# saugns/saugns

Hardware: AMD Instinct MI355X
Metric: mono samples/sec/GPU @ N voices (depth-3 FM) (higher is better)
Workload: dtype f32 (f64 table interpolation, u32 phase)

## Files before the change

### __graft_entry__.py

```python
import os
import subprocess
import sys

ROOT = os.path.dirname(os.path.abspath(__file__))
if ROOT not in sys.path:
    sys.path.insert(0, ROOT)


def build():
    import saugns_amd
    saugns_amd.build(force=False)
    subprocess.check_call(["make", "-s", "-C", os.path.join(ROOT, "tests", "seqexec")])
    subprocess.check_call(["make", "-s", "-C", os.path.join(ROOT, "tests", "hooks")])
    subprocess.check_call(["make", "-s", "-C", os.path.join(ROOT, "tests", "hooks_levels")])
    subprocess.check_call(["make", "-s", "-C", os.path.join(ROOT, "oracle"), "oracle"])
    subprocess.check_call(["make", "-s", "-C", os.path.join(ROOT, "oracle"), "ref"])
    subprocess.check_call(["make", "-s", "-C", os.path.join(ROOT, "oracle"), "hosts"])
    saugns_amd.lib()


def smoke():
    import numpy as np
    import saugns_amd as sa
    from saugns_amd import voicebank
    from oracle import pyoracle as po

    tabs = np.fromfile(os.path.join(ROOT, "tests", "golden", "piluts_ref.f32"),
                       dtype="<f4").reshape(12, 2048)
    sa.set_piluts(tabs)
    po.oracle_use_tables(tabs)
    po.oracle().ora_set_fastmath_forms(1)
    prg = voicebank.config3(n=16, seconds=1)
    want = po.oracle_render(prg.ptr, 44100, False)
    got = sa.Generator(prg, 44100).render(stereo=False)
    assert len(got) == len(want) == 44100, (len(got), len(want))
    diff = int(np.abs(got.astype(np.int32) - want.astype(np.int32)).max())
    assert diff == 0, f"GPU render differs from the oracle by {diff} LSB"
    print("smoke ok: 16 voices x depth-3 PM, 44100 frames, bit-exact vs oracle")
    from saugns_amd.api import POP_FMOD
    fm = [voicebank.Op("sin", freq=voicebank.Line(110.0 + 20 * k, goal=330.0, shape="exp"), time_ms=500,
                       mods={POP_FMOD: [voicebank.Op("sin", freq=5.0 + k, amp=20.0)]}) for k in range(8)]
    for name, p in (("8 FM voices with gliding carriers", voicebank.build_program(fm)),
                    ("16 feedback voices (config 5)", voicebank.config5(n=16, seconds=1))):
        want = po.oracle_render(p.ptr, 44100, False)
        got = sa.Generator(p, 44100).render(stereo=False)
        assert len(got) == len(want) and (got == want).all(), name
        print(f"smoke ok: {name}, {len(got)} frames, bit-exact vs oracle")


if __name__ == "__main__":
    build()
    if "--smoke" in sys.argv:
        smoke()
```

### saugns_amd/csrc/hip_backend.hip

```cpp
#include <hip/hip_runtime.h>
#include "hip_backend.h"
#include "launch_plan.h"
#include "sau_dev_ops.h"
#include <stdio.h>
#include <stdlib.h>
#include <string.h>
#include <deque>
#include <map>
#include <mutex>
#include <string>
#include <type_traits>
#include <vector>

namespace sauhip {

using namespace saudev;
using sauengine::BackendConfig;
using sauengine::tune_env;
using sauengine::SegmentDesc;
using namespace sauplan;

#include "k_common.h"
#include "k_block_loop.h"
#include "k_fast_types.h"
// ... 681 lines not shown
		if (getenv("SAU_AMD_DEBUG_DUO"))
			fprintf(stderr, "[sau-amd] duo %d: enabled %d look %d words_real %u FT %u rows_cf %u cub_ok %u tail %d may_scan %u of %u voices, lds %zu of %zu\n",
					(int)k.duo, (int)tun_.duo, fp.look != nullptr, fp.look_words_real, k.rows, k.rows_cf, fp.cub_ok, (int)j.tail_live, seg.n_may_scan, seg.n_voices,
					k.launch_lds(2, k.rows, false) + 1024, lim_.lds_limit);
		cfp.dyn_chunks = k.tasks_cf.dyn_chunks; cfp.dyn_static = k.tasks_cf.dyn_static;
		if (!k.duo && !launch_build(j, err, 0, k.rows_cf, k.grid_cf, &cfp, true, k.wide_cf)) j.launched = false;
		fp.mode = fp.sum_levels + 1; fp.only_multi = 0; fp.look_wpv = k.look_wpv; fp.look_groups = k.groups;
		fp.look_wpv_flags = k.look_wpv_flags;
		if (k.duo) {
			const size_t dlds = k.launch_lds(2, k.rows, false);
			if (!raise_lds_attr((const void *)duo_kernel, dlds, dev_, err)) return false;
			auto go = [&]() -> bool {
				void *da[] = {(void *)&fp, (void *)&cfp};
				return hipLaunchKernel((const void *)duo_kernel, dim3(lim_.fk_grid), dim3(1024), da, dlds, stream_) == hipSuccess;
			};
			if (!SpreadLaunchOrder::get().ordered(dev_, stream_, go)) j.launched = false;
		} else if (fp.look) {
			if (k.look_inside) {
				if (!launch_build(j, err, 2, k.rows, k.grid_look, nullptr, false, k.wide_look)) j.launched = false;
			} else if (!SpreadLaunchOrder::get().ordered(dev_, stream_, [&]() { return launch_build(j, err, 2, k.rows, k.grid_look, nullptr, false, k.wide_look); })) {
				j.launched = false;
			}
			if (fp.cub_ok) {
				const void *ck2 = fast_kernel_fn(2, FAST_CUB_ROWS, FK_CUB);
				const size_t lds2 = k.launch_lds(2, FAST_CUB_ROWS, false);
				if (!raise_lds_attr(ck2, lds2, dev_, err)) return false;
				auto go = [&]() -> bool {
					void *a2[] = {(void *)&fp};
					return hipLaunchKernel(ck2, dim3(k.grid_look), dim3(1024), a2, lds2, stream_) == hipSuccess;
				};
				if (k.look_inside ? !go() : !SpreadLaunchOrder::get().ordered(dev_, stream_, go)) j.launched = false;
			}
		}
		return true;
	}

	bool launch_sums_and_chains(Job &j, std::string &err) {
		const SegmentDesc &seg = j.seg;
		FastParams &fp = j.fp;
		if (fp.chain_rows && fp.chain_early_ok && !launch_early_chains(j, err)) return false;
		for (uint32_t pass = 1; pass <= fp.sum_levels && (!fp.look || seg.n_chain_rows); ++pass) {
			launch_fast(j, err, pass);
			hipLaunchKernelGGL(scan_kernel, dim3(seg.n_voices), dim3(64), 0, stream_, fp);
		}
		if (!fp.chain_rows) { launch_fast(j, err, fp.sum_levels + 1); return true; }
		return launch_chains(j, err);
	}

	bool launch_early_chains(Job &j, std::string &err) {
		FastParams &fp = j.fp;
		const uint32_t cgrid = j.fk.chain_grid;
		const size_t clds = chain_alone_lds((size_t)fp.n_ctabs * CHAIN_TAB_BYTES + CHAIN_IO_BYTES, cgrid);
		if (!raise_lds_attr((const void *)chain_kernel, clds, dev_, err)) return false;
		fp.chain_early = 1; fp.range_mode = 0;
		hipLaunchKernelGGL(chain_kernel, dim3(cgrid), dim3(192), clds, stream_, fp);
		const size_t rlds = chain_alone_lds(RCHAIN_LDS_BYTES, cgrid);
		if (!raise_lds_attr((const void *)rchain_kernel, rlds, dev_, err)) return false;
		hipLaunchKernelGGL(rchain_kernel, dim3(cgrid), dim3(RCHAIN_THREADS), rlds, stream_, fp);
		fp.chain_early = 0;
		return true;
	}

	bool launch_chains(Job &j, std::string &err) {
		const FastPlan &k = j.fk;
		FastParams &fp = j.fp;
		const uint32_t cgrid = k.chain_grid, n_chunks = k.chunks.n;
		const size_t clds = chain_alone_lds((size_t)fp.n_ctabs * CHAIN_TAB_BYTES + CHAIN_IO_BYTES, cgrid);
		if (!raise_lds_attr((const void *)chain_kernel, clds, dev_, err)) return false;
		TimedPair *tc = nullptr;
		if (n_chunks == 1) {
			tc = timing_on_ ? new_pair(0) : nullptr;
			fp.range_mode = 0;
			launch_fast(j, err, fp.sum_levels + 2);
			if (tc) (void)hipEventRecord(tc->a, stream_);
			hipLaunchKernelGGL(chain_kernel, dim3(cgrid), dim3(192), clds, stream_, fp);
			if (tc) (void)hipEventRecord(tc->b, stream_);
			launch_fast(j, err, fp.sum_levels + 1);
			return true;
		}
		if (!chain_stream_) {
			chain_stream_ = StreamPool::get().take(dev_, 1);
			if (!chain_stream_) {
				int lo = 0, hi = 0;
				(void)hipDeviceGetStreamPriorityRange(&lo, &hi);
				HIP_OK(hipStreamCreateWithPriority(&chain_stream_, hipStreamNonBlocking, hi));
			}
		}
		while (chain_ev_.size() < 2 * (size_t)n_chunks) {
			hipEvent_t e;
			HIP_OK(hipEventCreateWithFlags(&e, hipEventDisableTiming));
			chain_ev_.push_back(e);
		}
		tc = timing_on_ ? new_pair(0) : nullptr;
		const uint32_t *cb = k.chunks.cb;
		auto set_range = [&](FastParams &q, uint32_t mode, uint32_t c) {
			q.range_mode = mode; q.f_lo = cb[c]; q.f_hi = c + 1 == n_chunks ? 0xffffffffu : cb[c + 1];
		};
		for (uint32_t c = 0; c < n_chunks; ++c) {
			set_range(fp, 1, c);
			fp.range_last = c + 1 == n_chunks;
			launch_fast(j, err, fp.sum_levels + 2, k.pass_grid);
			HIP_OK(hipEventRecord(chain_ev_[2 * c], stream_));
			HIP_OK(hipStreamWaitEvent(chain_stream_, chain_ev_[2 * c], 0));
			FastParams cp = fp;
			set_range(cp, 1, c);
			if (tc && c == 0) (void)hipEventRecord(tc->a, chain_stream_);
			hipLaunchKernelGGL(chain_kernel, dim3(cgrid), dim3(192), clds, chain_stream_, cp);
			if (tc && c + 1 == n_chunks) (void)hipEventRecord(tc->b, chain_stream_);
			HIP_OK(hipEventRecord(chain_ev_[2 * c + 1], chain_stream_));
		}
		uint32_t mixed_blocks = 0;
		if (k.early_mix) hipLaunchKernelGGL(premix_kernel, dim3((j.seg.n_voices + 63) / 64), dim3(64), 0, stream_, fp);
		for (uint32_t c = 0; c < n_chunks; ++c) {
			HIP_OK(hipStreamWaitEvent(stream_, chain_ev_[2 * c + 1], 0));
			set_range(fp, 2, c);
			fp.range_last = c + 1 == n_chunks;
			launch_fast(j, err, fp.sum_levels + 1, c + 1 == n_chunks ? k.grid : k.pass_grid);
			if (k.early_mix && c + 1 < n_chunks && cb[c + 1] > 512) {
				const uint32_t hi = (cb[c + 1] - 512) / 256;
				if (hi > mixed_blocks) {
					MixParams mp = mix_params(j.seg, set_);
					mp.blk_lo = mixed_blocks; mp.blk_hi = hi;
					TimedPair *tm = timing_on_ ? new_pair(1) : nullptr;
					if (tm) (void)hipEventRecord(tm->a, stream_);
					hipLaunchKernelGGL((j.in.f32 ? mix_kernel_f32 : mix_kernel), dim3(hi - mixed_blocks, j.seg.n_streams), dim3(256), 0, stream_, mp);
					if (tm) (void)hipEventRecord(tm->b, stream_);
					mixed_blocks = hi;
				}
			}
		}
		j.early_mixed_blocks = mixed_blocks;
		fp.range_mode = 0; fp.f_lo = 0; fp.f_hi = 0; fp.range_last = 0;
		return true;
	}

	bool launch_closed_form(Job &j, std::string &err) {
		const SegmentDesc &seg = j.seg;
		const FastPlan &k = j.fk;
		FastParams &fp = j.fp;
		fp.dyn_chunks = k.tasks.dyn_chunks; fp.dyn_static = k.tasks.dyn_static; fp.dyn_small = k.tasks.dyn_small;
		if (k.queues) {
			fp.inmix_flags = k.inmix_flags;
			fp.inmix_div_s = k.div.s; fp.inmix_div_m = k.div.m;
			if (k.inmix) {
				fp.inmix_stream = set_.mstreams.p;
				fp.inmix_pcm_offset = seg.pcm_offset;
				hipLaunchKernelGGL(premix_kernel, dim3((seg.n_voices + 63) / 64), dim3(64), 0, stream_, fp);
				j.inmix_live = true;
			}
		}
		if (k.inner != INNER_NONE) {
			const bool lm = k.inner == INNER_LANE_MAJOR;
			const void *ik = fast_kernel_fn(0, 12, FK_WIDE | FK_INNER | (lm ? FK_LANEMAJOR : 0u));
			const size_t lds = k.launch_lds(0, k.rows, true);
			FastParams ep = fp;
			ep.mode = 0; ep.edge_only = 1; ep.dyn_static = 1; ep.dyn_chunks = 2; ep.dyn_small = 0; ep.inmix_flags = 0;
			if (!launch_build(j, err, 0, k.rows, k.grid_edge, &ep, false, true)) j.launched = false;
			fp.mode = 0;
			void *iargs[] = {(void *)&fp};
			if (!raise_lds_attr(ik, lds, dev_, err)) return false;
			HIP_OK(hipLaunchKernel(ik, dim3(k.grid), dim3(1024), iargs, lds, stream_));
			if (inner_report_) fprintf(stderr, "[sau-amd] inner: %s, %u voices\n", lm ? "lane-major" : "row-major", seg.n_voices);
		} else {
			if (inner_report_) fprintf(stderr, "[sau-amd] inner: none (rows %u, wide %d, chunks %u), %u voices\n", k.rows, k.wide_cf ? 1 : 0, fp.dyn_chunks, seg.n_voices);
			launch_fast(j, err, 0);
		}
		fp.dyn_chunks = 0; fp.inmix_flags = 0; fp.dyn_small = 0;
		return true;
	}

	bool launch_cub(Job &j, std::string &err) {
		if (!j.fp.cub_ok) return true;
		const FastPlan &k = j.fk;
		FastParams q = k.main_build == 2 ? j.cfp : j.fp;
		q.n_fast = k.n_fast_cf; q.rows = FAST_CUB_ROWS; q.mode = 0; q.only_multi = 0;
		q.dyn_chunks = k.tasks_cub.dyn_chunks; q.dyn_static = k.tasks_cub.dyn_static;
		const size_t qlds = k.launch_lds(0, FAST_CUB_ROWS, false, true);
		const void *ck = fast_kernel_fn(0, FAST_CUB_ROWS, FK_CUB);
		if (!raise_lds_attr(ck, qlds, dev_, err)) return false;
		void *qargs[] = {(void *)&q};
		HIP_OK(hipLaunchKernel(ck, dim3(k.grid_cub), dim3(1024), qargs, qlds, stream_));
		return true;
	}

	bool launch_repair(Job &j, std::string &err) {
		const FastPlan &k = j.fk;
		const size_t rlds = k.launch_lds(0, k.rows_repair, k.wide_cf, k.main_build == 2);
		FastParams rpar = k.main_build == 2 ? j.cfp : j.fp;
		rpar.mode = 0;
		const void *rk = repair_kernel_fn(k.rows_repair, k.wide_cf);
		if (!rk) {
			err = "internal error: no repair_kernel build with " + std::to_string(k.rows_repair) + " rows per pass in this form";
			return false;
		}
		if (!raise_lds_attr(rk, rlds, dev_, err)) return false;
		j.fp.mode = 0;
		void *rargs[] = {(void *)&rpar};
		HIP_OK(hipLaunchKernel(rk, dim3(k.grid_repair), dim3(1024), rargs, rlds, stream_));
		return true;
	}

	bool launch_finalize(Job &j, std::string &err) {
		const SegmentDesc &seg = j.seg;
		TimedPair *tz = timing_on_ ? new_pair(3) : nullptr;
		if (tz) (void)hipEventRecord(tz->a, stream_);
		hipLaunchKernelGGL(finalize_kernel, dim3((unsigned)(((size_t)seg.n_voices * j.fp.max_ops * 8 + 63) / 64)), dim3(64), 0,
				stream_, j.fp);
		if (tz) (void)hipEventRecord(tz->b, stream_);
		HIP_OK(hipGetLastError());
		if (debug_ && j.fk.use_fast) {
			(void)hipStreamSynchronize(stream_);
			FastInfo fi0;
			(void)hipMemcpy(&fi0, finfo_.p, sizeof fi0, hipMemcpyDeviceToHost);
			fprintf(stderr, "[sau-amd] fast: voice 0 total %u H %u bail %u steps %u seq %u; n_fast %u rows %u\n",
					fi0.total, fi0.H, fi0.bail, fi0.n_fsteps, fi0.seq, j.fk.n_fast, j.fk.rows);
			std::vector<FastStep> fs(fi0.n_fsteps < 64 ? fi0.n_fsteps : 64);
			if (!fs.empty()) (void)hipMemcpy(fs.data(), fsteps_.p, fs.size() * sizeof(FastStep), hipMemcpyDeviceToHost);
			for (size_t i = 0; i < fs.size(); ++i)
				fprintf(stderr, "[sau-amd]   step %zu kind %u flags %#x which %u dep %u out %d pm %d fpm %d amp %d aux %d type %#x inc %u ac %g fc %g ramp %u\n",
						i, fs[i].kind & 0xff, (fs[i].kind >> 8) & 0xff, (fs[i].kind >> 16) & 0xff, fs[i].kind >> 24,
						(int)fs[i].out_off, (int)fs[i].pm_off, (int)fs[i].fpm_off, (int)fs[i].amp_off, (int)fs[i].aux_off,
						fs[i].type, fs[i].inc, fs[i].ac, fs[i].fc, fs[i].ramp);
		}
		return true;
	}

	bool launch_block_loop(Job &j, std::string &err) {
		const SegmentDesc &seg = j.seg;
		const BlockLoopPlan &b = j.bl;
		RenderParams &rp = j.rp;
		rp.team_bytes = (uint32_t)b.team_bytes;
		memcpy(rp.tab_of_wave, b.tabs.tab_of_wave, sizeof rp.tab_of_wave);
		memcpy(rp.wave_of_tab, b.tabs.wave_of_tab, sizeof rp.wave_of_tab);
		rp.voices = voices_.p; rp.steps = steps_.p; rp.op_ids = op_ids_.p; rp.ops = ops_.p;
		rp.vout = set_.vout.p; rp.pan = set_.pan.p; rp.vinfo = set_.vinfo.p;
		rp.g_c23 = tables_->c23; rp.g_c01 = tables_->c01;
		rp.row_stride = row_stride_; rp.seg_len = seg.len;
		rp.n_slots = seg.n_slots; rp.max_ops = seg.max_ops; rp.n_tabs = b.tabs.n;
		rp.max_steps = seg.max_steps; rp.n_main = seg.n_main;
		memcpy(rp.wc, wconst_, sizeof wconst_);
		rp.fast_done = fdone_.p; rp.worklist = worklist_.p; rp.work_count = work_count_.p;
		j.block_grid = b.grid(seg, j.fk.use_fast);
		if (b.HB) {
			const size_t stride = ((size_t)seg.n_slots * 64 * sizeof(float) + (size_t)seg.max_ops * sizeof(DevOp) +
				(size_t)seg.max_steps * sizeof(Step) + 255) / 256 * 256 / sizeof(float);
			if (stride > 0xffffffffu) { err = "voice too large (block buffers + operator records beyond 16 GiB)"; return false; }
			if (!big_slots_.ensure((size_t)j.block_grid * stride, err)) return false;
			rp.big_slots = big_slots_.p; rp.big_stride = (uint32_t)stride;
		}
		if (!wait_for_predecessor(err)) return false;
		TimedPair *tp = timing_on_ ? new_pair(0) : nullptr;
		if (tp) (void)hipEventRecord(tp->a, stream_);
		const void *fn = render_kernel_fn(b.W, b.T, b.V, b.HB);
		if (!fn) { err = "internal error: no render_kernel build of this geometry"; return false; }
		if (!raise_lds_attr(fn, b.lds, dev_, err)) return false;
		void *args[] = {(void *)&rp};
		HIP_OK(hipLaunchKernel(fn, dim3(j.block_grid), dim3(64 * b.W * b.V), args, b.lds, stream_));
		HIP_OK(hipGetLastError());
		if (tp) (void)hipEventRecord(tp->b, stream_);
		if (debug_) debug_dump("after render", seg, j.block_grid);
		return true;
	}

	bool launch_mixer(Job &j, std::string &err) {
		const SegmentDesc &seg = j.seg;
		const uint32_t max_write = j.in.max_write;
		const Mixer which = plan_mixer(seg, tun_, j.in, pcm_pitch(), j.inmix_live, j.early_mixed_blocks);
		if (which == MIX_NONE) return true;
		MixParams mp = mix_params(seg, set_);
		mp.early_blocks = j.early_mixed_blocks;
		mp.inmix = j.inmix_live ? inmix_ctl_.p : nullptr;
		mp.tail_ok = j.tail_live ? tail_ok_.p : nullptr;
		TimedPair *tm = timing_on_ ? new_pair(1) : nullptr;
		if (tm) (void)hipEventRecord(tm->a, stream_);
		switch (which) {
		case MIX_FEW_F32: hipLaunchKernelGGL(mix_few_kernel_f32, dim3((max_write + 1023) / 1024, seg.n_streams), dim3(256), 0, stream_, mp); break;
		case MIX_F32: hipLaunchKernelGGL(mix_kernel_f32, dim3((max_write + 255) / 256, seg.n_streams), dim3(256), 0, stream_, mp); break;
		case MIX_FEW: hipLaunchKernelGGL(mix_few_kernel, dim3((max_write + 1023) / 1024, seg.n_streams), dim3(256), 0, stream_, mp); break;
		case MIX_64: hipLaunchKernelGGL(mix_kernel64, dim3((max_write + 63) / 64, seg.n_streams), dim3(64), 0, stream_, mp); break;
		default: hipLaunchKernelGGL(mix_kernel, dim3((max_write + 255) / 256, seg.n_streams), dim3(256), 0, stream_, mp); break;
		}
		HIP_OK(hipGetLastError());
		if (tm) (void)hipEventRecord(tm->b, stream_);
		if (mp.inmix && inmix_report_) report_inmix(mp, seg.n_voices, max_write);
		return true;
	}

	void report_inmix(const MixParams &mp, uint32_t n_voices, uint32_t max_write) {
		std::vector<uint32_t> h(INMIX_WORDS);
		uint32_t g[2] = {0, 0};
		(void)hipStreamSynchronize(stream_);
		(void)hipMemcpy(h.data(), mp.inmix, INMIX_WORDS * sizeof(uint32_t), hipMemcpyDeviceToHost);
		(void)hipMemcpy(g, work_count_.p, sizeof g, hipMemcpyDeviceToHost);
		const uint32_t nch = h[INMIX_NCH] < INMIX_MAX_CHUNKS ? h[INMIX_NCH] : INMIX_MAX_CHUNKS, tpc = h[INMIX_TPC];
		uint32_t tiles = 0, whole = 0, all = 0;
		for (uint32_t k = 0; k < nch; ++k) {
			uint32_t lo_f = k * h[INMIX_CF], hi_f = lo_f + h[INMIX_CF];
			if (k >= h[INMIX_NCH1]) { lo_f = h[INMIX_BASE] + (k - h[INMIX_NCH1]) * h[INMIX_CFS]; hi_f = lo_f + h[INMIX_CFS]; }
			else if (hi_f > h[INMIX_BASE]) hi_f = h[INMIX_BASE];
			if (hi_f > max_write) hi_f = max_write;
			const uint32_t tk = hi_f > lo_f ? (hi_f - lo_f + INMIX_TILE - 1) / INMIX_TILE : 0u;
			uint32_t c = 0;
			for (uint32_t j = 0; j < tk && j < tpc && j < INMIX_MAX_TPC; ++j) c += (h[INMIX_CHUNK + INMIX_LINE * k + INMIX_BITS + (j >> 5)] >> (j & 31u)) & 1u;
			tiles += c; whole += c == tk ? 1u : 0u; all += tk;
		}
		fprintf(stderr, "[sau-amd] inmix: voices %u frames %u chunks %u x %u frames, tiles %u of %u, chunks mixed whole %u, guard %u %u\n",
				n_voices, max_write, nch, h[INMIX_CF], tiles, all, whole, g[0], g[1]);
// ... 428 lines not shown
```

### saugns_amd/csrc/k_fast_group_lm.h

```cpp
		const int j0 = l * T;
		const int t0 = (int)(cg * GF) - (int)H + j0;
		const uint32_t om = ((1u << T) - 1u) & ~((1u << min(max((int)H - j0, 0), T)) - 1u);
		auto prev32 = [&](const uint32_t *x, int k) -> uint32_t { return k > 0 ? x[k - 1] : lane_prev(x[T - 1]); };
		auto prev64 = [&](const double *x, int k) -> double { return k > 0 ? x[k - 1] : lane_prev(x[T - 1]); };
		const bool quads = ((cg * GF - H) & 3u) == 0;
		auto store_row = [&](float *row, const float *x, const bool nt) {
			uint32_t o = om;
			asm volatile("" : "+v"(o));
			if (quads) {
#pragma unroll
				for (int q = 0; q < T / 4; ++q) {
					const uint32_t oq = (o >> (4 * q)) & 15u;
					if (oq == 15u) {
						const fk_f32x4 v4 = {x[4 * q], x[4 * q + 1], x[4 * q + 2], x[4 * q + 3]};
						fk_f32x4 *p = (fk_f32x4 *)(row + t0 + 4 * q);
						if (nt) FK_VSTORE(p, v4); else *p = v4;
					} else if (oq != 0u) {
#pragma unroll
						for (int u = 0; u < 4; ++u)
							if ((oq >> u) & 1u) { if (nt) FK_VSTORE(&row[t0 + 4 * q + u], x[4 * q + u]); else row[t0 + 4 * q + u] = x[4 * q + u]; }
					}
				}
			} else {
#pragma unroll
				for (int k = 0; k < T; ++k)
					if ((o >> k) & 1u) { if (nt) FK_VSTORE(&row[t0 + k], x[k]); else row[t0 + k] = x[k]; }
			}
		};
		uint32_t held_rows = 0;
		bool held_far = false;
		for (uint32_t si = 0; si < n_fsteps; ++si) {
			const FastStep f = load_step_uniform(fsteps + si);
			const uint32_t kind = f.kind & 0xff;
			const uint32_t flags = (f.kind >> 8) & 0xff;
			if (kind == ST_OSC) {
				const uint32_t type = f.type & 0xff;
				const bool wave_env = (flags & SF_WAVE_ENV) != 0;
				const bool layer = (flags & SF_LAYER) != 0;
				const bool to_voice = ((f.kind >> 16) & OX_VOICE) != 0;
				float s[T];
				if (type == OT_WAVE) {
					const bool has_pm = f.pm_off != ~0u, has_fpm = f.fpm_off != ~0u;
					const int p_min = (int)H - (int)(f.kind >> 24) + 1;
					const int nd = min(max(p_min - j0, 0), T);
					const uint32_t dm = ((1u << T) - 1u) & ~((1u << nd) - 1u);
					bool done = false;
					if (FK_COMMON && f.tab >= 0 && !has_fpm && !(f.ramp & 2)) {
						uint32_t ph[T];
						{
							uint32_t acc = f.phase0 + f.inc * (uint32_t)(t0 + 1);
#pragma unroll
							for (int k = 0; k < T; ++k) { ph[k] = acc; acc += f.inc; }
						}
						bool ok = true;
						if (has_pm) {
							float pm[T];
							bool big = false;
#pragma unroll
							for (int k = 0; k < T; ++k) {
								pm[k] = slots[f.pm_off + k * 64];
								big |= !(fabsf(pm[k]) < 0x1p20f);
							}
							ok = !__any(big);
#pragma unroll
							for (int k = 0; k < T; ++k) ph[k] += rint32w_p31_small(pm[k]);
						}
						if (ok) {
							const uint32_t ltab = tabs + (uint32_t)f.tab * FkTab<WIDE>::BYTES;
							double Is[T];
#pragma unroll
							for (int k = 0; k < T; ++k) Is[k] = fk_poly(fk_entry<WIDE>(ltab, ph[k]), ph[k]);
							if (FK_CONSTD && !has_pm && f.inc != 0) {
								const double x = (double)div_f32_normal(f.diff_scale, (float)(int32_t)f.inc);
#pragma unroll
								for (int k = 0; k < T; ++k)
									s[k] = (float)((Is[k] - prev64(Is, k)) * x + (double)f.diff_offset);
								done = true;
							} else {
								uint32_t dmin = 0xffffffffu;
#pragma unroll
								for (int k = 0; k < T; ++k) {
									uint32_t pp = prev32(ph, k);
									if (k == 0) asm("" : "+v"(pp));
									const int32_t d = (int32_t)(ph[k] - pp);
									dmin = min(dmin, (uint32_t)d);
									s[k] = wosc_diff(Is[k], prev64(Is, k), d, f.diff_scale, f.diff_offset);
								}
								done = true;
								if (__any(dmin == 0u)) {
									uint32_t hz = 0;
#pragma unroll
									for (int k = 0; k < T; ++k) hz |= ph[k] == prev32(ph, k) ? 1u << k : 0u;
									done = !__any((hz & dm) != 0u);
								}
							}
						}
					}
					if (!done) {
						uint32_t ph[T];
						double Is[T];
						float fv[T];
						{
							uint32_t acc = f.phase0 + f.inc * (uint32_t)(t0 + 1);
#pragma unroll
							for (int k = 0; k < T; ++k) { ph[k] = acc; acc += f.inc; fv[k] = f.fc; }
						}
						if (has_pm && !has_fpm) {
							float pm[T];
							bool big = false;
#pragma unroll
							for (int k = 0; k < T; ++k) {
								pm[k] = slots[f.pm_off + k * 64];
								big |= !(fabsf(pm[k]) < 0x1p20f);
							}
							if (!__any(big)) {
#pragma unroll
								for (int k = 0; k < T; ++k) ph[k] += rint32w_p31_small(pm[k]);
							} else {
#pragma unroll
								for (int k = 0; k < T; ++k) ph[k] += rint32w_p31(pm[k]);
							}
						} else if (has_pm || has_fpm) {
							float pm[T], fpm[T];
#pragma unroll
							for (int k = 0; k < T; ++k) { pm[k] = 0.f; fpm[k] = 0.f; }
							if (has_pm) {
#pragma unroll
								for (int k = 0; k < T; ++k) pm[k] = slots[f.pm_off + k * 64];
							}
							if (has_fpm) {
#pragma unroll
								for (int k = 0; k < T; ++k) fpm[k] = slots[f.fpm_off + k * 64];
							}
							if (has_pm) {
#pragma unroll
								for (int k = 0; k < T; ++k) ph[k] += pm_offset32(true, true, pm[k], fpm[k], fv[k]);
							} else {
#pragma unroll
								for (int k = 0; k < T; ++k) ph[k] += pm_offset32(false, true, 0.f, fpm[k], fv[k]);
							}
						}
						if (f.tab >= 0) {
							const uint32_t ltab = tabs + (uint32_t)f.tab * FkTab<WIDE>::BYTES;
#pragma unroll
							for (int k = 0; k < T; ++k) Is[k] = fk_poly(fk_entry<WIDE>(ltab, ph[k]), ph[k]);
						} else {
							const uint32_t wave = (f.type >> 8) & 0xff;
							const HerpC23 *g23 = P.g_c23 + (size_t)wave * WAVE_LEN;
							const HerpC01 *g01 = P.g_c01 + (size_t)wave * WAVE_LEN;
#pragma unroll
							for (int k = 0; k < T; ++k) {
								const uint32_t ind = ph[k] >> SLEN_BITS;
								Is[k] = herp_poly(g23[ind], g01[ind], ph[k]);
							}
						}
						uint32_t hz = 0;
						if (FK_CONSTD && !has_pm && !has_fpm && f.inc != 0) {
							const double x = (double)div_f32_normal(f.diff_scale, (float)(int32_t)f.inc);
#pragma unroll
							for (int k = 0; k < T; ++k) {
								const double pIs = prev64(Is, k);
								s[k] = (float)((Is[k] - pIs) * x + (double)f.diff_offset);
							}
						} else {
#pragma unroll
							for (int k = 0; k < T; ++k) {
								const uint32_t pph = prev32(ph, k);
								const double pIs = prev64(Is, k);
								const int32_t d = (int32_t)(ph[k] - pph);
								hz |= d == 0 ? 1u << k : 0u;
								s[k] = wosc_diff(Is[k], pIs, d, f.diff_scale, f.diff_offset);
							}
						}
						uint32_t held = hz & dm;
						if (__any(held != 0u)) {
							uint32_t src = dm & ~held;
							auto in_lane = [&]() {
#pragma unroll
								for (int k = 1; k < T; ++k)
									if (((held >> k) & 1u) && ((src >> (k - 1)) & 1u)) { s[k] = s[k - 1]; held &= ~(1u << k); src |= 1u << k; }
							};
							in_lane();
							for (int it = 0; it < 64; ++it) {
								const float sp = __shfl_up(s[T - 1], 1);
								const uint32_t okp = ((uint32_t)__shfl_up((int)src, 1) >> (T - 1)) & 1u;
								bool changed = false;
								if ((held & 1u) && okp && l > 0) { s[0] = sp; held &= ~1u; src |= 1u; changed = true; in_lane(); }
								if (!__any(changed)) break;
							}
							const int jm = min(32, 64 - (int)FAST_REPAIR_SHIFT - (int)H);
							if (held) {
								const int j = j0 + (int)__builtin_ctz(held);
								rep[1] = ((uint32_t)(j % 64 - p_min) << 24) | ((uint32_t)(j / 64) << 20) | (si << 12) | (cg & 0xfff);
							}
							const int nf = jm + p_min - j0;
							const bool far = nf <= 0 ? held != 0u : nf < T ? (held >> nf) != 0u : false;
							if (__any(far)) held_far = true;
							if (jm > 0) {
								unsigned long long run = 0;
#pragma unroll
								for (int L = 0; L * T < 64; ++L)
									run |= (unsigned long long)(uint32_t)__builtin_amdgcn_readlane((int)held, L) << (L * T);
								held_rows |= (uint32_t)((run >> p_min) & ((1ull << jm) - 1ull));
							}
						}
					}
				} else if (type == OT_RASEG) {
					const bool rate2x = (f.type >> 17) & 1;
					const float phase_scale = rate2x ? 0x1p31f * 2 : 0x1p31f;
					const RasParams rp = ras_params((uint32_t)f.tab & 0xff, ((uint32_t)f.tab >> 8) & 0xffff,
							f_bits(f.diff_scale), f_bits(f.diff_offset), ((uint32_t)f.tab >> 24) & 0x7f);
					const unsigned long long inc64 = ((unsigned long long)f.prev_phase << 32) | f.inc;
					const unsigned long long cp0 = (unsigned long long)__double_as_longlong(f.prev_Is);
					const bool has_pm = f.pm_off != ~0u, has_fpm = f.fpm_off != ~0u;
#pragma unroll
					for (int k = 0; k < T; ++k) {
						unsigned long long cp = cp0 + inc64 * (unsigned long long)(long long)(t0 + k);
						if (has_pm || has_fpm)
							cp += (unsigned long long)pm_offset(has_pm, has_fpm,
									has_pm ? slots[f.pm_off + k * 64] : 0.f,
									has_fpm ? slots[f.fpm_off + k * 64] : 0.f, f.fc, phase_scale);
						uint32_t cyc;
						float phf;
						ras_split(cp, cyc, phf);
						s[k] = ras_sample(rp, cyc, phf, true, false);
					}
				} else if (type == OT_NOISE) {
					const uint32_t nz = (f.type >> 8) & 0xff;
					const uint32_t n0 = f.phase0;
#pragma unroll
					for (int k = 0; k < T; ++k) {
						const uint32_t n = n0 + (uint32_t)(t0 + k);
						if (nz == NZ_vi) {
							uint32_t s1 = ranfast32(n);
							uint32_t s0 = ranfast32(n - 1);
							s[k] = fscalei((s1 / 2) - (s0 / 2), 0x1p-31f);
						} else if (nz == NZ_bv) {
							int32_t s1 = noise_bv_term(n);
							int32_t s0 = noise_bv_term(n - 1);
							s[k] = (float)(s1 - s0);
						} else {
							s[k] = noise_stateless(nz, n);
						}
					}
				} else {
#pragma unroll
					for (int k = 0; k < T; ++k) s[k] = f.fc;
				}
				float r[T];
				if (f.amp_off != ~0u) {
#pragma unroll
					for (int k = 0; k < T; ++k) r[k] = slots[f.amp_off + k * 64];
				} else if (f.ramp & 1) {
					const FastLine fl = load_line_uniform(flines + si);
#pragma unroll
					for (int k = 0; k < T; ++k) r[k] = fast_line_value(fl, t0 + k);
				} else {
#pragma unroll
					for (int k = 0; k < T; ++k) r[k] = f.ac;
				}
				if (layer) {
#pragma unroll
					for (int k = 0; k < T; ++k)
						r[k] = mix_combine(slots[f.out_off + k * 64], s[k], r[k], wave_env, true);
				} else if (wave_env) {
#pragma unroll
					for (int k = 0; k < T; ++k) r[k] = mix_combine(0.f, s[k], r[k], true, false);
				} else {
#pragma unroll
					for (int k = 0; k < T; ++k) r[k] = s[k] * r[k];
				}
				if (to_voice) {
					store_row(vrow, r, true);
				} else {
#pragma unroll
					for (int k = 0; k < T; ++k) slots[f.out_off + k * 64] = r[k];
				}
			} else if (kind == ST_LINE) {
				if (f.ramp) {
					FastLine fl;
					fl.goal_len = 0; fl.hold = f.ac; fl.pad = 0;
					fl.sw = sweep_setup(LN_sah, 0.f, 0.f, 0, 1);
					if (f.ramp & 1) fl = load_line_uniform(flines + si);
#pragma unroll
					for (int k = 0; k < T; ++k) slots[f.out_off + k * 64] = fast_line_value(fl, t0 + k);
				} else {
#pragma unroll
					for (int k = 0; k < T; ++k) slots[f.out_off + k * 64] = f.ac;
				}
			} else if (kind == ST_LERP) {
				const bool end_const = f.aux_off == ~0u;
#pragma unroll
				for (int k = 0; k < T; ++k) {
					float pv = slots[f.out_off + k * 64];
					pv += ((end_const ? f.fc : slots[f.aux_off + k * 64]) - pv) * slots[f.pm_off + k * 64];
					slots[f.out_off + k * 64] = pv;
				}
			} else if (kind == ST_VOICE) {
				float x[T];
#pragma unroll
				for (int k = 0; k < T; ++k) x[k] = slots[f.out_off + k * 64];
				store_row(vrow, x, true);
				if (prow) {
#pragma unroll
					for (int k = 0; k < T; ++k) x[k] = f.pm_off != ~0u ? slots[f.pm_off + k * 64] : f.pan;
					store_row(prow, x, false);
				}
			}
		}
		if (held_rows || held_far) {
			bool noted = false;
			if (P.repair_on && !held_far && (int)(cg * GF) - (int)H >= (int)FAST_REPAIR_SHIFT) {
				uint32_t at = 0;
				if (l == 0) at = atomicAdd(&rep[0], 1u);
				at = uni(at);
				if (at < FAST_MAX_REPAIR) {
					if (l == 0) {
						rep[2 + 2 * at] = cg;
						rep[3 + 2 * at] = held_rows;
						atomicOr(&P.pass_flags[FAST_MAX_LEVELS], 1u);
						atomicOr(&P.work_count[1], 2u);
					}
					noted = true;
				}
			}
			if (!noted) zero_acc = 1;
		}
```

### saugns_amd/csrc/launch_plan.h

```cpp
#ifndef SAU_LAUNCH_PLAN_H
#define SAU_LAUNCH_PLAN_H

#include "engine.h"
#include "sau_dev_math.h"
#include <string.h>

namespace sauplan {

using namespace saudev;
using sauengine::SegmentDesc;

#ifndef FK_GRID
#define FK_GRID 256
#endif
constexpr uint32_t FAST_TAB_BYTES = (uint32_t)(WAVE_LEN * (sizeof(HerpC23) + sizeof(HerpC01))), FAST_TAB_BYTES_WIDE = 65536u;
constexpr uint32_t FAST_MAX_SCAN = 8;
constexpr uint32_t LOOK_LDS_BYTES = FAST_MAX_SCAN * 2 * 64 * sizeof(unsigned long long);
constexpr uint32_t FAST_MAX_LEVELS = 3;
constexpr uint32_t FAST_CUB_ROWS = 4;
constexpr uint32_t FAST_LISTS = 5;
constexpr uint32_t INMIX_NSMALL = 8;
#ifndef SAU_CHAIN_BATCH_FRAMES
#define SAU_CHAIN_BATCH_FRAMES 32
#endif
// ... 197 lines not shown
			return all ? (full < 512 ? full : 512) : 2;
		}
		return all ? (seg.n_voices < 1024 ? seg.n_voices : 1024) : 16;
	}
};
inline BlockLoopPlan plan_block_loop(const SegmentDesc &seg, const Tuning &tun, const DeviceLimits &dev) {
	BlockLoopPlan p;
	p.W = tun.geo ? 4 : 8; p.T = tun.geo ? 4 : 2;
	auto team_size = [&](uint32_t w, uint32_t t) {
		size_t b = p.HB ? MISC_BYTES + 64
			: (size_t)w * 64 * t * sizeof(float) * seg.n_slots + (size_t)seg.max_ops * sizeof(DevOp) +
			MISC_BYTES + (size_t)seg.max_steps * sizeof(Step) + 64;
		return (b + 15) & ~(size_t)15;
	};
	if (tun.multi_min && seg.n_voices >= tun.multi_min && (seg.serial || tun.multi_min == 1)) {
		const size_t need_tab = seg.wave_mask ? BLOCK_TAB_BYTES : 0;
		const uint32_t mt = tun.multi_teams;
		for (uint32_t t : {4u, 3u, 2u, 1u})
			if (mt * team_size(1, t) + need_tab <= dev.lds_limit) { p.W = 1; p.T = t; p.V = mt; break; }
	}
	if (p.V == 1 && team_size(p.W, p.T) > dev.lds_limit) { p.W = 1; p.T = 1; }
	if (p.V == 1 && p.W == 1 && team_size(1, 1) > dev.lds_limit) p.HB = true;
	p.team_bytes = team_size(p.W, p.T);
	const size_t fixed = p.team_bytes * p.V;
	if (fixed > dev.lds_limit) { p.ok = false; return p; }
	size_t budget = dev.lds_limit / 2 > fixed ? dev.lds_limit / 2 - fixed : 0;
	if (p.V > 1) budget = dev.lds_limit - fixed;
	if (budget < BLOCK_TAB_BYTES && dev.lds_limit - fixed >= BLOCK_TAB_BYTES) budget = BLOCK_TAB_BYTES;
	p.tabs = map_tables(seg.wave_mask, budget / BLOCK_TAB_BYTES);
	p.lds = p.tabs.n * BLOCK_TAB_BYTES + fixed;
	return p;
}

struct ChainChunks {
	uint32_t n = 1;
	uint32_t cb[34];
	bool short_last = false;
};
inline ChainChunks chain_chunk_bounds(uint32_t len, const Tuning &tun) {
	ChainChunks k;
	uint32_t n = tun.chain_chunks ? tun.chain_chunks : (len + tun.chain_chunk_frames - 1) / tun.chain_chunk_frames;
	if (n > 32) n = 32;
	while (n > 1 && len / n < 4096) --n;
	if (n < 1) n = 1;
	k.short_last = !tun.chain_chunks && tun.short_last_chunk && n >= 4 && n < 32 && len > 8 * 4096u;
	const uint32_t tail = k.short_last ? 4096u : 0u;
	const uint32_t body = tail ? (len - tail) & ~255u : len;
	const uint32_t clen0 = ((body + n - 1) / n + 255) & ~255u;
	for (uint32_t c = 0; c <= n; ++c) k.cb[c] = (unsigned long long)c * clen0 < body ? c * clen0 : body;
	if (tail) { ++n; k.cb[n] = len; }
	uint32_t m = 0;
	for (uint32_t c = 0; c < n; ++c)
		if (k.cb[c + 1] > k.cb[c]) { k.cb[m] = k.cb[c]; ++m; k.cb[m] = k.cb[c + 1]; }
	if (m) n = m;
	k.n = n;
	return k;
}

struct Tasks { uint32_t dyn_chunks = 0, dyn_static = 0, dyn_small = 0; };
inline uint32_t task_groups(const SegmentDesc &seg, const Tuning &tun) {
	const uint32_t S = seg.max_steps ? seg.max_steps : 1;
	uint32_t G = tun.dyn_groups;
	if (G * S < tun.dyn_floor) G = (tun.dyn_floor + S - 1) / S;
	return G;
}
inline Tasks plan_tasks(const SegmentDesc &seg, const Tuning &tun, uint32_t n_groups, uint32_t grid) {
	Tasks q;
	const uint32_t waves = grid * 16;
	const uint32_t G = task_groups(seg, tun);
	const uint32_t k_dyn = (n_groups + G - 1) / G;
	if (tun.dyn && (unsigned long long)seg.n_voices * k_dyn >= (unsigned long long)tun.dyn_min_tasks * waves) {
		q.dyn_chunks = k_dyn ? k_dyn : 1;
		q.dyn_static = 0;
	} else {
		uint32_t k = waves / seg.n_voices;
		if (k > n_groups) k = n_groups;
		q.dyn_chunks = k ? k : 1;
		q.dyn_static = 1;
	}
	return q;
}
inline Tasks static_tasks(const SegmentDesc &seg, uint32_t n_groups, uint32_t grid) {
	Tasks q;
	uint32_t k = grid * 16 / seg.n_voices;
	if (k > n_groups) k = n_groups;
	q.dyn_chunks = k ? k : 1; q.dyn_static = 1;
	return q;
}
struct MagicDiv { uint32_t m = 0, s = 0; };
inline MagicDiv magic_div(uint32_t d) {
	MagicDiv q;
	while ((1ull << q.s) < d) ++q.s;
	q.m = (uint32_t)(((1ull << (32 + q.s)) / d) + 1ull - (1ull << 32));
	return q;
}
inline uint32_t magic_quotient(uint32_t q, MagicDiv d) {
	if (d.s == 0) return q;
	const uint32_t t = (uint32_t)(((unsigned long long)q * d.m) >> 32);
	return (t + ((q - t) >> 1)) >> (d.s - 1);
}

enum Inner : uint32_t { INNER_NONE = 0, INNER_ROW_MAJOR = 1, INNER_LANE_MAJOR = 2 };
enum Mixer : uint32_t { MIX_NONE = 0, MIX_FEW_F32, MIX_F32, MIX_FEW, MIX_64, MIX_256 };

struct FastPlan {
	bool use_fast = false;
	bool seq_ok = false;
	bool look_split = false;
	int main_build = 0;
	uint32_t fmax_steps = 0, n_fast = 0, n_fast_cf = 0;
	uint32_t rows = 2;
	uint32_t rows_multi = 2;
	uint32_t rows_cf = 2;
	uint32_t rows_lean = 4;
	bool lean_on = false;
	TableMap tabs;
	uint32_t n_want = 0;
	bool wide_cf = false;
	bool wide_look = false;
	bool cub_ok = false;
	uint32_t sum_levels = 2;
	uint32_t scan_groups = 0;
	bool scan = false;
	bool look = false;
	size_t look_words = 0;
	bool look_words_real = false;
	uint32_t look_wpv = 1;
	bool look_inside = true;
	uint32_t look_wpv_flags = 0;
	bool inc_rows = false;
	uint32_t inc_stride = 0;
	bool chains = false;
	uint32_t chain_stride = 0, chain_grid = 0;
	TableMap ctabs;
	ChainChunks chunks;
	uint32_t pass_grid = 0;
	bool early_mix = false;
	bool split_cf = false, duo = false, tailmix = false;
	bool queues = false;
	bool inmix = false;
	uint32_t inmix_flags = 0;
	MagicDiv div;
	Inner inner = INNER_NONE;
	Tasks tasks, tasks_cf, tasks_cub;
	uint32_t groups = 0, groups_cf = 0;
	uint32_t grid = 1, grid_cf = 1, grid_look = 1, grid_edge = 1, grid_cub = 1, grid_repair = 1;
	uint32_t rows_repair = 2;

	void drop_chains() { chains = false; lean_on = false; }
	size_t launch_lds(int build, uint32_t r, bool wide, bool cf = false) const {
		return tabs.n * (size_t)(wide ? FAST_TAB_BYTES_WIDE : FAST_TAB_BYTES) + 16 * buf_area(cf ? n_fast_cf : n_fast, r, fmax_steps) +
			(build == 2 ? LOOK_LDS_BYTES : 0);
	}
};

inline void plan_rows(FastPlan &p, const SegmentDesc &seg, const Tuning &tun, const DeviceLimits &dev) {
	p.fmax_steps = seg.max_steps < 64 ? seg.max_steps : 64;
	uint32_t FT = tun.fast_rows;
	p.look_split = tun.seq && seg.may_scan && tun.two_pass && tun.lookback && tun.look_rows != 0 && seg.n_voices >= tun.look_min_voices;
	if (tun.seq && seg.may_scan && FT > 4 && !p.look_split) FT = 4;
	if (p.look_split && FT > tun.look_rows) FT = rows_at_most(tun.look_rows);
	p.seq_ok = tun.seq && seg.may_scan;
	p.n_fast = p.seq_ok && seg.n_fast_full > seg.n_fast ? seg.n_fast_full : seg.n_fast;
	p.n_fast_cf = seg.n_fast;
	p.n_want = n_waves_used(seg.wave_mask);
	auto area_of = [&](uint32_t t) { return buf_area(p.n_fast, t, p.fmax_steps); };
	const size_t look_lds = p.look_split ? LOOK_LDS_BYTES : 0;
	while (FT > 2 && !fits_lds(dev, seg.wave_mask ? 1 : 0, FAST_TAB_BYTES, area_of(FT), look_lds)) FT = fewer_rows(FT);
	{
		uint32_t t = FT;
		while (t > 4 && !fits_lds(dev, p.n_want, FAST_TAB_BYTES, area_of(t), look_lds)) t = fewer_rows(t);
		if (fits_lds(dev, p.n_want, FAST_TAB_BYTES, area_of(t), look_lds)) FT = t;
	}
	p.use_fast = tun.fast && fits_lds(dev, 0, 0, area_of(FT), look_lds);
	p.rows = FT;
	p.rows_multi = FT > 4 && p.seq_ok ? 4 : FT;
	p.tabs = map_tables(seg.wave_mask, p.use_fast ? tabs_that_fit(dev.lds_limit, 16 * area_of(FT) + look_lds + 1024, FAST_TAB_BYTES) : 0);
	const uint32_t ft = p.tabs.n;
	const bool all_wide_ok = tun.wide_tabs && tun.more_rows && ft > 0 && ft == p.n_want && seg.max_steps >= 2;
	if (p.use_fast && !p.seq_ok && all_wide_ok && FT == 8)
		for (uint32_t t : {12u, 10u})
			if (t <= tun.more_rows && fits_lds(dev, ft, FAST_TAB_BYTES_WIDE, area_of(t))) { p.rows = p.rows_multi = t; break; }
	p.split_cf = p.use_fast && p.seq_ok && p.look_split;
	auto area_cf = [&](uint32_t t) { return buf_area(p.n_fast_cf, t, p.fmax_steps); };
	p.rows_cf = 2;
	if (p.split_cf) {
		for (uint32_t t : {8u, 6u, 5u, 4u})
			if (t <= tun.fast_rows && fits_lds(dev, ft, FAST_TAB_BYTES, area_cf(t))) { p.rows_cf = t; break; }
		if (p.rows_cf == 8 && all_wide_ok)
			for (uint32_t t : {12u, 10u})
				if (t <= tun.more_rows && fits_lds(dev, ft, FAST_TAB_BYTES_WIDE, area_cf(t))) { p.rows_cf = t; break; }
	}
	p.cub_ok = p.use_fast && seg.maybe_cub && fits_lds(dev, ft, FAST_TAB_BYTES, area_cf(FAST_CUB_ROWS)) &&
		(!p.look_split || fits_lds(dev, ft, FAST_TAB_BYTES, area_of(FAST_CUB_ROWS), LOOK_LDS_BYTES));
	p.rows_lean = 4;
	for (uint32_t t : {6u, 5u})
		if (t <= tun.fast_rows && t <= tun.lean_rows && fits_lds(dev, ft, FAST_TAB_BYTES, area_of(t))) { p.rows_lean = t; break; }
	p.main_build = !p.seq_ok ? 0 : p.look_split ? 2 : 1;
	auto wide_fits = [&](uint32_t rows, size_t area) {
		return tun.wide_tabs && (rows == 8 || rows == 6 || rows == 10 || rows == 12) && ft > 0 && ft == p.n_want && seg.max_steps >= 2 &&
			fits_lds(dev, ft, FAST_TAB_BYTES_WIDE, area);
	};
	p.wide_cf = p.main_build == 2 ? wide_fits(p.rows_cf, area_cf(p.rows_cf)) : p.main_build == 0 && wide_fits(p.rows, area_of(p.rows));
	p.wide_look = tun.wide_tabs && tun.wide_look && p.rows == 8 && ft > 0 && ft == p.n_want &&
		fits_lds(dev, ft, FAST_TAB_BYTES_WIDE, area_of(p.rows), LOOK_LDS_BYTES);
	p.sum_levels = seg.sum_levels >= FAST_MAX_LEVELS ? FAST_MAX_LEVELS : 2u;
}

inline void plan_sums(FastPlan &p, const SegmentDesc &seg, const Tuning &tun, const DeviceLimits &dev) {
	if (p.seq_ok && tun.two_pass) {
		p.scan_groups = seg.len / (32 * p.rows_multi) + 2;
		p.scan = !p.look_split || seg.n_chain_rows;
		p.look = p.look_split && seg.n_look_rows;
	}
	if (p.look) {
		const uint32_t groups = row_groups(seg.len, p.rows);
		unsigned long long wpv = ((unsigned long long)dev.fk_grid * 16) / seg.n_voices;
		if (wpv > 64) wpv = 64;
		if (wpv > groups) wpv = groups;
		if (wpv < 1) wpv = 1;
		auto is_inside = [&](unsigned long long w) { return w <= 16 && (16 % w) == 0 && !tun.look_no_lds; };
		p.look_words = (size_t)seg.n_look_rows * 2 * p.scan_groups;
		p.look_words_real = p.look_words * sizeof(unsigned long long) <= ((size_t)1 << 30);
		if (!p.look_words_real && !is_inside(wpv) && !tun.look_no_lds)
			wpv = wpv > 16 ? 16 : wpv > 8 ? 8 : wpv > 4 ? 4 : 2;
		p.look_wpv = (uint32_t)wpv;
		p.look_inside = !p.look_words_real && is_inside(wpv);
	}
	p.inc_stride = (seg.len + 63) & ~63u;
	p.inc_rows = tun.inc_rows && p.use_fast && p.scan && seg.n_inc_rows && seg.len <= sauengine::CHAIN_SEG &&
		(size_t)seg.n_inc_rows * 2 * p.inc_stride * sizeof(uint32_t) <= ((size_t)1 << 30);
}

inline void plan_chains(FastPlan &p, const SegmentDesc &seg, const Tuning &tun, const DeviceLimits &dev, const PlanInputs &in) {
	p.chains = tun.chain && p.use_fast && p.scan && seg.serial && seg.n_chain_rows &&
		seg.len <= sauengine::chain_seg_frames(seg.n_chain_rows, in.chain_budget);
	p.chain_stride = (seg.len + 63) & ~63u;
	p.ctabs = map_tables(seg.wave_mask, tabs_that_fit(dev.lds_limit, CHAIN_IO_BYTES + 1024, CHAIN_TAB_BYTES));
	p.lean_on = p.chains && tun.lean &&
		fits_lds(dev, p.tabs.n, FAST_TAB_BYTES, buf_area(p.n_fast, p.rows_lean, p.fmax_steps));
	p.chain_grid = (seg.n_chain_slots + 63) / 64;
	if (p.chains) p.chunks = chain_chunk_bounds(seg.len, tun);
	p.pass_grid = p.chunks.n > 1 && p.grid + p.chain_grid > dev.fk_grid ? (dev.fk_grid > p.chain_grid + 32 ? dev.fk_grid - p.chain_grid : 32) : p.grid;
	p.early_mix = tun.early_mix && in.max_write && !p.cub_ok && !(tun.mix_few && in.max_rows <= 8 && seg.n_streams >= 8);
}

inline void plan_split(FastPlan &p, const SegmentDesc &seg, const Tuning &tun, const DeviceLimits &dev, const PlanInputs &in) {
	const uint32_t ft = p.tabs.n;
	p.tailmix = p.look && p.rows == 8 && tun.tailmix && !in.f32 && in.max_write && !p.cub_ok && seg.len < (1u << 30) &&
		tun.mix_few && in.max_rows <= 8 && seg.n_streams >= 8 && (seg.pcm_offset & 3u) == 0 && (in.pcm_row & 3u) == 0;
	p.groups_cf = row_groups(seg.len, p.rows_cf);
	p.grid_cf = group_grid(seg.n_voices, p.groups_cf, dev.fk_grid);
	p.duo = tun.duo && p.look && p.look_words_real && p.rows == 8 && p.rows_cf == 8 && !p.cub_ok && !p.tailmix &&
		!p.wide_look && !p.wide_cf && fits_lds(dev, ft, FAST_TAB_BYTES, buf_area(p.n_fast, p.rows, p.fmax_steps), LOOK_LDS_BYTES);
	p.tasks_cf = plan_tasks(seg, tun, p.groups_cf, p.duo ? (dev.fk_grid + 1) / 2 : p.grid_cf);
	p.look_wpv_flags = (tun.look_no_lds ? 1u : 0u) | (tun.look_withhold ? 2u : 0u) | (tun.look_spread ? 4u : 0u);
	if (p.duo) p.look_wpv_flags |= (tun.duo_lw << 8) | (tun.duo_prio << 12);
	p.grid_look = wave_grid((unsigned long long)seg.n_voices * (p.look_words_real ? (p.groups < 64 ? p.groups : 64) : p.look_wpv), dev.fk_grid);
}

inline void plan_closed_form(FastPlan &p, const SegmentDesc &seg, const Tuning &tun, const DeviceLimits &dev, const PlanInputs &in) {
	if (p.main_build == 0) p.tasks = plan_tasks(seg, tun, p.groups, p.grid);
	p.queues = tun.xcd_queues && dev.eight_xcds && p.main_build == 0 && !p.tasks.dyn_static && p.tasks.dyn_chunks >= 16 && !p.cub_ok;
	if (p.queues) {
		p.inmix_flags = 64u;
		if (tun.inmix_taper) {
			const uint32_t G = task_groups(seg, tun);
			const uint32_t small = G / 4 ? G / 4 : 1;
			if (p.groups >= 32 * G + INMIX_NSMALL * small) {
				p.tasks.dyn_small = small;
				p.tasks.dyn_chunks = (p.groups - INMIX_NSMALL * small + G - 1) / G + INMIX_NSMALL;
			}
		}
		p.div = magic_div(seg.n_voices);
		p.inmix = tun.inmix && !in.f32 && seg.n_streams == 1 && in.max_write && seg.n_voices >= tun.inmix_min_voices &&
			seg.max_steps >= tun.inmix_min_steps && in.row_stride < (1u << 24);
		if (p.inmix)
			p.inmix_flags = 64u | 32u | (seg.stereo ? 1u : 0u) | (seg.swap_bytes ? 2u : 0u) | (tun.inmix_dry ? 4u : 0u) | ((tun.inmix_at & 15u) << 8);
	}
	if (tun.inner && p.main_build == 0 && p.wide_cf && p.rows == 12 && p.tasks.dyn_chunks >= 3)
		p.inner = tun.lanemajor ? INNER_LANE_MAJOR : INNER_ROW_MAJOR;
	p.grid_edge = wave_grid(2ull * seg.n_voices, dev.fk_grid);
}

inline FastPlan plan_fast(const SegmentDesc &seg, const Tuning &tun, const DeviceLimits &dev, const PlanInputs &in) {
	FastPlan p;
	plan_rows(p, seg, tun, dev);
	plan_sums(p, seg, tun, dev);
	p.groups = row_groups(seg.len, p.rows);
	p.grid = group_grid(seg.n_voices, p.groups, dev.fk_grid);
	plan_chains(p, seg, tun, dev, in);
	if (p.use_fast && p.main_build == 2) plan_split(p, seg, tun, dev, in);
	if (p.use_fast && !p.scan) plan_closed_form(p, seg, tun, dev, in);
	const uint32_t g4 = row_groups(seg.len, FAST_CUB_ROWS);
	p.grid_cub = group_grid(seg.n_voices, g4, dev.fk_grid);
	p.tasks_cub = static_tasks(seg, g4, p.grid_cub);
	p.rows_repair = p.main_build == 2 ? p.rows_cf : p.rows;
	p.grid_repair = wave_grid(seg.n_voices, 64);
	return p;
}

inline Mixer plan_mixer(const SegmentDesc &seg, const Tuning &tun, const PlanInputs &in, size_t pcm_pitch, bool inmix_live,
		uint32_t early_blocks) {
	if (!in.max_write) return MIX_NONE;
	const bool few = tun.mix_few && in.max_rows <= 8 && seg.n_streams >= 8;
	const bool few_f32_aligned = (pcm_pitch & 15u) == 0 && (seg.pcm_offset & (seg.stereo ? 1u : 3u)) == 0;
	if (in.f32) return few && few_f32_aligned ? MIX_FEW_F32 : MIX_F32;
	if (few && (seg.pcm_offset & 3u) == 0 && (in.pcm_row & 3u) == 0) return MIX_FEW;
	if (inmix_live && !early_blocks && tun.mix64) return MIX_64;
	return MIX_256;
}

constexpr uint32_t LEVELS_THREADS = 256;
constexpr uint32_t LEVELS_SWEEP_F32 = LEVELS_THREADS * 4, LEVELS_SWEEP_S16 = LEVELS_THREADS * 8;
constexpr uint32_t LEVELS_WG_SAMPLES = 16384;
static_assert(LEVELS_WG_SAMPLES % LEVELS_SWEEP_S16 == 0 && LEVELS_WG_SAMPLES % LEVELS_SWEEP_F32 == 0, "a block is whole sweeps (and begins on an even sample, on 16 bytes)");
constexpr uint32_t LEVELS_MAX_ROWS = 65535;
struct LevelsPlan {
	bool ok = false;
	uint32_t blocks = 0;
	uint32_t rows = 0;
	uint32_t finish_grid = 0;
	size_t parts = 0;
};
inline LevelsPlan plan_levels(uint64_t max_frames, uint32_t channels, size_t n_rows) {
	LevelsPlan p;
	const uint64_t samples = max_frames * channels;
	const uint64_t blocks = (samples + LEVELS_WG_SAMPLES - 1) / LEVELS_WG_SAMPLES;
	if (n_rows > LEVELS_MAX_ROWS || blocks > 0x7fffffffull || max_frames > (~(uint64_t)0 >> 2)) return p;
	p.ok = true;
	p.blocks = (uint32_t)blocks;
	p.rows = (uint32_t)n_rows;
	p.finish_grid = (uint32_t)((n_rows + 63) / 64);
	p.parts = (size_t)n_rows * (size_t)blocks;
	return p;
}

}
#endif
```

Baseline: 240.1 million.

## Keep lane-major inner chain in registers and drop its LDS slot buffer

The lane-major inner kernel now carries the single fast-buffer chain in a per-lane register block instead of reading and writing LDS slots. Steps it cannot handle with one buffer set a fallback flag and are skipped. The planner picks lane-major only when there is one fast buffer, and the launch requests LDS for the tables only. Less LDS per block may allow more resident blocks and removes the slot traffic, but it narrows when lane-major applies and leans on the fallback path for other step kinds.

```diff
diff --git a/__graft_entry__.py b/__graft_entry__.py
--- a/__graft_entry__.py
+++ b/__graft_entry__.py
@@ -13,6 +13,7 @@
     subprocess.check_call(["make", "-s", "-C", os.path.join(ROOT, "tests", "seqexec")])
     subprocess.check_call(["make", "-s", "-C", os.path.join(ROOT, "tests", "hooks")])
     subprocess.check_call(["make", "-s", "-C", os.path.join(ROOT, "tests", "hooks_levels")])
+    subprocess.check_call(["make", "-s", "-C", os.path.join(ROOT, "tests", "hooks_plan")])
     subprocess.check_call(["make", "-s", "-C", os.path.join(ROOT, "oracle"), "oracle"])
     subprocess.check_call(["make", "-s", "-C", os.path.join(ROOT, "oracle"), "ref"])
     subprocess.check_call(["make", "-s", "-C", os.path.join(ROOT, "oracle"), "hosts"])
diff --git a/saugns_amd/csrc/hip_backend.hip b/saugns_amd/csrc/hip_backend.hip
--- a/saugns_amd/csrc/hip_backend.hip
+++ b/saugns_amd/csrc/hip_backend.hip
@@ -857,7 +857,7 @@
 		if (k.inner != INNER_NONE) {
 			const bool lm = k.inner == INNER_LANE_MAJOR;
 			const void *ik = fast_kernel_fn(0, 12, FK_WIDE | FK_INNER | (lm ? FK_LANEMAJOR : 0u));
-			const size_t lds = k.launch_lds(0, k.rows, true);
+			const size_t lds = k.inner_lds();
 			FastParams ep = fp;
 			ep.mode = 0; ep.edge_only = 1; ep.dyn_static = 1; ep.dyn_chunks = 2; ep.dyn_small = 0; ep.inmix_flags = 0;
 			if (!launch_build(j, err, 0, k.rows, k.grid_edge, &ep, false, true)) j.launched = false;
diff --git a/saugns_amd/csrc/k_fast_group_lm.h b/saugns_amd/csrc/k_fast_group_lm.h
--- a/saugns_amd/csrc/k_fast_group_lm.h
+++ b/saugns_amd/csrc/k_fast_group_lm.h
@@ -29,13 +29,24 @@
 		};
 		uint32_t held_rows = 0;
 		bool held_far = false;
+		float blk[T];
 		for (uint32_t si = 0; si < n_fsteps; ++si) {
 			const FastStep f = load_step_uniform(fsteps + si);
 			const uint32_t kind = f.kind & 0xff;
 			const uint32_t flags = (f.kind >> 8) & 0xff;
+			int t0s = t0;
+			asm volatile("" : "+v"(t0s));
+			{
+				const uint32_t o1 = f.out_off + 1u, p1 = f.pm_off + 1u, q1 = f.fpm_off + 1u, a1 = f.amp_off + 1u;
+				uint32_t two = 0;
+				if (kind == ST_OSC) two = o1 | a1 | (p1 + q1) | (flags & SF_WAVE_ENV);
+				else if (kind == ST_LINE) two = o1;
+				else if (kind == ST_VOICE) two = o1 | (p1 << 1);
+				else if (kind == ST_LERP) two = 2u;
+				if (two > 1u) { zero_acc = 1; continue; }
+			}
 			if (kind == ST_OSC) {
 				const uint32_t type = f.type & 0xff;
-				const bool wave_env = (flags & SF_WAVE_ENV) != 0;
 				const bool layer = (flags & SF_LAYER) != 0;
 				const bool to_voice = ((f.kind >> 16) & OX_VOICE) != 0;
 				float s[T];
@@ -58,7 +69,7 @@
 							bool big = false;
 #pragma unroll
 							for (int k = 0; k < T; ++k) {
-								pm[k] = slots[f.pm_off + k * 64];
+								pm[k] = blk[k];
 								big |= !(fabsf(pm[k]) < 0x1p20f);
 							}
 							ok = !__any(big);
@@ -110,7 +121,7 @@
 							bool big = false;
 #pragma unroll
 							for (int k = 0; k < T; ++k) {
-								pm[k] = slots[f.pm_off + k * 64];
+								pm[k] = blk[k];
 								big |= !(fabsf(pm[k]) < 0x1p20f);
 							}
 							if (!__any(big)) {
@@ -120,25 +131,9 @@
 #pragma unroll
 								for (int k = 0; k < T; ++k) ph[k] += rint32w_p31(pm[k]);
 							}
-						} else if (has_pm || has_fpm) {
-							float pm[T], fpm[T];
-#pragma unroll
-							for (int k = 0; k < T; ++k) { pm[k] = 0.f; fpm[k] = 0.f; }
-							if (has_pm) {
-#pragma unroll
-								for (int k = 0; k < T; ++k) pm[k] = slots[f.pm_off + k * 64];
-							}
-							if (has_fpm) {
-#pragma unroll
-								for (int k = 0; k < T; ++k) fpm[k] = slots[f.fpm_off + k * 64];
-							}
-							if (has_pm) {
-#pragma unroll
-								for (int k = 0; k < T; ++k) ph[k] += pm_offset32(true, true, pm[k], fpm[k], fv[k]);
-							} else {
-#pragma unroll
-								for (int k = 0; k < T; ++k) ph[k] += pm_offset32(false, true, 0.f, fpm[k], fv[k]);
-							}
+						} else if (has_fpm) {
+#pragma unroll
+							for (int k = 0; k < T; ++k) ph[k] += pm_offset32(false, true, 0.f, blk[k], fv[k]);
 						}
 						if (f.tab >= 0) {
 							const uint32_t ltab = tabs + (uint32_t)f.tab * FkTab<WIDE>::BYTES;
@@ -215,11 +210,11 @@
 					const bool has_pm = f.pm_off != ~0u, has_fpm = f.fpm_off != ~0u;
 #pragma unroll
 					for (int k = 0; k < T; ++k) {
-						unsigned long long cp = cp0 + inc64 * (unsigned long long)(long long)(t0 + k);
+						unsigned long long cp = cp0 + inc64 * (unsigned long long)(long long)(t0s + k);
 						if (has_pm || has_fpm)
 							cp += (unsigned long long)pm_offset(has_pm, has_fpm,
-									has_pm ? slots[f.pm_off + k * 64] : 0.f,
-									has_fpm ? slots[f.fpm_off + k * 64] : 0.f, f.fc, phase_scale);
+									has_pm ? blk[k] : 0.f,
+									has_fpm ? blk[k] : 0.f, f.fc, phase_scale);
 						uint32_t cyc;
 						float phf;
 						ras_split(cp, cyc, phf);
@@ -230,7 +225,7 @@
 					const uint32_t n0 = f.phase0;
 #pragma unroll
 					for (int k = 0; k < T; ++k) {
-						const uint32_t n = n0 + (uint32_t)(t0 + k);
+						const uint32_t n = n0 + (uint32_t)(t0s + k);
 						if (nz == NZ_vi) {
 							uint32_t s1 = ranfast32(n);
 							uint32_t s0 = ranfast32(n - 1);
@@ -250,22 +245,18 @@
 				float r[T];
 				if (f.amp_off != ~0u) {
 #pragma unroll
-					for (int k = 0; k < T; ++k) r[k] = slots[f.amp_off + k * 64];
+					for (int k = 0; k < T; ++k) r[k] = blk[k];
 				} else if (f.ramp & 1) {
 					const FastLine fl = load_line_uniform(flines + si);
 #pragma unroll
-					for (int k = 0; k < T; ++k) r[k] = fast_line_value(fl, t0 + k);
+					for (int k = 0; k < T; ++k) r[k] = fast_line_value(fl, t0s + k);
 				} else {
 #pragma unroll
 					for (int k = 0; k < T; ++k) r[k] = f.ac;
 				}
 				if (layer) {
 #pragma unroll
-					for (int k = 0; k < T; ++k)
-						r[k] = mix_combine(slots[f.out_off + k * 64], s[k], r[k], wave_env, true);
-				} else if (wave_env) {
-#pragma unroll
-					for (int k = 0; k < T; ++k) r[k] = mix_combine(0.f, s[k], r[k], true, false);
+					for (int k = 0; k < T; ++k) r[k] = mix_combine(blk[k], s[k], r[k], false, true);
 				} else {
 #pragma unroll
 					for (int k = 0; k < T; ++k) r[k] = s[k] * r[k];
@@ -274,7 +265,7 @@
 					store_row(vrow, r, true);
 				} else {
 #pragma unroll
-					for (int k = 0; k < T; ++k) slots[f.out_off + k * 64] = r[k];
+					for (int k = 0; k < T; ++k) blk[k] = r[k];
 				}
 			} else if (kind == ST_LINE) {
 				if (f.ramp) {
@@ -283,27 +274,17 @@
 					fl.sw = sweep_setup(LN_sah, 0.f, 0.f, 0, 1);
 					if (f.ramp & 1) fl = load_line_uniform(flines + si);
 #pragma unroll
-					for (int k = 0; k < T; ++k) slots[f.out_off + k * 64] = fast_line_value(fl, t0 + k);
-				} else {
-#pragma unroll
-					for (int k = 0; k < T; ++k) slots[f.out_off + k * 64] = f.ac;
-				}
-			} else if (kind == ST_LERP) {
-				const bool end_const = f.aux_off == ~0u;
-#pragma unroll
-				for (int k = 0; k < T; ++k) {
-					float pv = slots[f.out_off + k * 64];
-					pv += ((end_const ? f.fc : slots[f.aux_off + k * 64]) - pv) * slots[f.pm_off + k * 64];
-					slots[f.out_off + k * 64] = pv;
+					for (int k = 0; k < T; ++k) blk[k] = fast_line_value(fl, t0s + k);
+				} else {
+#pragma unroll
+					for (int k = 0; k < T; ++k) blk[k] = f.ac;
 				}
 			} else if (kind == ST_VOICE) {
-				float x[T];
-#pragma unroll
-				for (int k = 0; k < T; ++k) x[k] = slots[f.out_off + k * 64];
-				store_row(vrow, x, true);
+				store_row(vrow, blk, true);
 				if (prow) {
-#pragma unroll
-					for (int k = 0; k < T; ++k) x[k] = f.pm_off != ~0u ? slots[f.pm_off + k * 64] : f.pan;
+					float x[T];
+#pragma unroll
+					for (int k = 0; k < T; ++k) x[k] = f.pan;
 					store_row(prow, x, false);
 				}
 			}
diff --git a/saugns_amd/csrc/launch_plan.h b/saugns_amd/csrc/launch_plan.h
--- a/saugns_amd/csrc/launch_plan.h
+++ b/saugns_amd/csrc/launch_plan.h
@@ -373,6 +373,9 @@
 		return tabs.n * (size_t)(wide ? FAST_TAB_BYTES_WIDE : FAST_TAB_BYTES) + 16 * buf_area(cf ? n_fast_cf : n_fast, r, fmax_steps) +
 			(build == 2 ? LOOK_LDS_BYTES : 0);
 	}
+	size_t inner_lds() const {
+		return inner == INNER_LANE_MAJOR ? tabs.n * (size_t)FAST_TAB_BYTES_WIDE : launch_lds(0, rows, true);
+	}
 };
 
 inline void plan_rows(FastPlan &p, const SegmentDesc &seg, const Tuning &tun, const DeviceLimits &dev) {
@@ -500,7 +503,7 @@
 			p.inmix_flags = 64u | 32u | (seg.stereo ? 1u : 0u) | (seg.swap_bytes ? 2u : 0u) | (tun.inmix_dry ? 4u : 0u) | ((tun.inmix_at & 15u) << 8);
 	}
 	if (tun.inner && p.main_build == 0 && p.wide_cf && p.rows == 12 && p.tasks.dyn_chunks >= 3)
-		p.inner = tun.lanemajor ? INNER_LANE_MAJOR : INNER_ROW_MAJOR;
+		p.inner = tun.lanemajor && p.n_fast == 1 ? INNER_LANE_MAJOR : INNER_ROW_MAJOR;
 	p.grid_edge = wave_grid(2ull * seg.n_voices, dev.fk_grid);
 }
 
```

After: 246.8 million, median of 6. +2.8%, better.
